# audeering/opensmile

Measured on NVIDIA H100. Metric: LLD frames/sec (16kHz, 25ms/10ms), higher is better.
Workload: dtype f32

## Files before the change

### opensmile_b200/csrc/lld_common.cuh

```cuda
#pragma once
#include <cstdio>

#include "fft_radix.cuh"
#include "kernels.cuh"

namespace osm {

struct SmemLayout {
  int zbuf, samp, raw, rawPcm, mbar, winLut, tw, splitTw, melCoef, melRange, dctCos, dctLift, eql, melS, ring;
  int total;
  int sampFloats, rawPcmBytes;
};

__host__ __device__ inline int align_up(int x, int a) { return (x + a - 1) / a * a; }

constexpr int kLeadFrames = 8;

__host__ __device__ inline SmemLayout make_layout(const LldParams &p, int M, int F)
{
  SmemLayout L;
  int o = 0;
  L.zbuf = o; o += M * F * 8;
  const int S = p.frameStep + p.sPad;
  L.sampFloats = align_up((F - 1) * S + p.frameSize + ((p.frameSize - 1) / p.frameStep) * p.sPad + 2, 4);
  L.samp = o; o += L.sampFloats * 4;
  L.raw = o; o += F * 4;
  o = align_up(o, 16);
  L.rawPcmBytes = align_up(16 + (kLeadFrames + (F - 1) * p.frameStep + p.frameSize) * p.nChan * 2, 16);
  L.rawPcm = o; o += L.rawPcmBytes;
  L.mbar = o; o += 16;
  L.winLut = o; o += M * 16;
  L.tw = o; o += p.twCount * 8;
  L.splitTw = o; o += (M / 2 + 1) * 8;
  o = align_up(o, 16);
  L.melCoef = o; o += (p.melVCount + 4) * 8;
  L.melRange = o; o += 2 * (p.nBands + 2) * 4;
  o = align_up(o, 16);
  L.dctCos = o; o += max(p.dctRows * p.dctStride, p.opKind == 0 ? p.nBands * 16 : 0) * 4;
  L.dctLift = o; o += p.nStat * 4;
  L.eql = o; o += (p.opKind == 1 ? p.nBands : 0) * 4;
  o = align_up(o, 16);
  if (L.sampFloats >= p.nBands * F) L.melS = L.samp;
  else { L.melS = o; o += p.nBands * F * 4; }
  L.ring = o; o += p.nStat * 2 * F * 4;
  L.total = align_up(o, 16);
  return L;
}

__device__ __forceinline__ float div32767(float x)
{
  const float rc = 3.0518509447574615e-05f;
  const float q0 = __fmul_rn(x, rc);
  const float r = __fmaf_rn(-q0, 32767.0f, x);
  return __fmaf_rn(r, rc, q0);
}

#define OSM_COLD __noinline__
template <bool F32>
__device__ __forceinline__ float pcm_to_float_generic(const int16_t *s, int nChan)
{
  if constexpr (F32) return *reinterpret_cast<const float *>(s);
  float tmp = (float)s[0];
  for (int c = 1; c < nChan; c++) tmp = __fadd_rn(tmp, (float)s[c]);
  if (nChan == 1) return div32767(tmp);
  if (nChan == 2) return div32767(tmp * 0.5f);
  return __fdiv_rn(__fdiv_rn(tmp, (float)nChan), 32767.0f);
}
template <bool F32>
static __device__ OSM_COLD float pcm_to_float_slow(const int16_t *s, int nChan) { return pcm_to_float_generic<F32>(s, nChan); }

__device__ __forceinline__ uint32_t smem_u32(const void *p) { return (uint32_t)__cvta_generic_to_shared(p); }

__device__ __forceinline__ void mbar_init(uint64_t *bar, int count)
{
  asm volatile("mbarrier.init.shared::cta.b64 [%0], %1;" ::"r"(smem_u32(bar)), "r"(count));
  asm volatile("fence.mbarrier_init.release.cluster;" ::: "memory");
}
__device__ __forceinline__ void mbar_expect_tx(uint64_t *bar, uint32_t bytes)
{
  asm volatile("mbarrier.arrive.expect_tx.shared::cta.b64 _, [%0], %1;" ::"r"(smem_u32(bar)), "r"(bytes) : "memory");
}
__device__ __forceinline__ void bulk_g2s(void *dst, const void *src, uint32_t bytes, uint64_t *bar)
{
  asm volatile("cp.async.bulk.shared::cluster.global.mbarrier::complete_tx::bytes [%0], [%1], %2, [%3];"
               ::"r"(smem_u32(dst)), "l"(src), "r"(bytes), "r"(smem_u32(bar)) : "memory");
}
__device__ __forceinline__ void mbar_wait(uint64_t *bar, uint32_t parity)
{
  asm volatile(
      "{\n"
      ".reg .pred p;\n"
      "LAB_WAIT:\n"
      "mbarrier.try_wait.parity.shared::cta.b64 p, [%0], %1;\n"
      "@p bra LAB_DONE;\n"
      "bra LAB_WAIT;\n"
      "LAB_DONE:\n"
      "}\n" ::"r"(smem_u32(bar)), "r"(parity) : "memory");
}

struct ChunkCtx {
  int utt, a, b;
  int T;
  int s0;
  int sEnd;
  int nT;
  int tile0;
  long long uo;
  long long row0;
};

template <int F>
__device__ __forceinline__ ChunkCtx load_chunk(const LldParams &p, int chunk)
{
  ChunkCtx c;
  const ChunkRef cr = p.chunks[chunk];
  c.utt = cr.utt; c.a = cr.a; c.b = cr.b; c.tile0 = cr.tile0;
  c.uo = p.uttOff[cr.utt];
  const long long Ls = p.uttOff[cr.utt + 1] - c.uo;
  c.T = (int)((Ls - p.frameSize) / p.frameStep + 1);
  c.s0 = max(cr.a - p.halo, 0);
  c.sEnd = min(cr.b + p.halo, c.T);
  c.nT = (c.sEnd - c.s0 + F - 1) / F;
  c.row0 = p.rowOff[cr.utt];
  return c;
}

__device__ __forceinline__ int chunk_run_begin(const LldParams &p, int g)
{
  const long long w = (long long)p.chunks[0].w0 + (long long)g * p.ctaTiles;
  int lo = 0, hi = p.nChunks;
  while (lo < hi) {
    const int mid = (lo + hi) >> 1;
    if (p.chunks[mid].w0 < w) lo = mid + 1;
    else hi = mid;
  }
  return lo;
}

struct TileGeom {
  int fs;
  int nf;
  int count;
  int lead;
  int mis;
  uint32_t bytes;
  const char *src;
};

template <int F>
__device__ __forceinline__ TileGeom tile_geom(const LldParams &p, const ChunkCtx &c, int j)
{
  TileGeom g;
  g.fs = c.s0 + j * F;
  g.nf = min(F, c.sEnd - g.fs);
  const long long s0 = (long long)g.fs * p.frameStep;
  g.count = (g.nf - 1) * p.frameStep + p.frameSize;
  g.lead = (s0 > 0) ? kLeadFrames : 0;
  const char *a = reinterpret_cast<const char *>(p.pcm + (c.uo + s0 - g.lead) * p.nChan);
  g.mis = (int)(reinterpret_cast<uintptr_t>(a) & 15);
  g.src = a - g.mis;
  g.bytes = (uint32_t)align_up(g.mis + (g.lead + g.count) * p.nChan * 2, 16);
  return g;
}

__device__ __forceinline__ float div_exact(float x, float d, float rcp)
{
  const float ax = fabsf(x);
  if (rcp != 0.f && ax > 1e-30f && ax < 1e30f) {
    const float q0 = __fmul_rn(x, rcp);
    const float r = __fmaf_rn(-q0, d, x);
    return __fmaf_rn(r, rcp, q0);
  }
  return __fdiv_rn(x, d);
}

__device__ __forceinline__ int win_navail(int t, int n0, int c0, int Tprev)
{
  return (t < c0) ? Tprev : min(n0 + (t - c0) + 1, Tprev);
}

template <int M, int F, int NVW, int R, int MS, bool FIRST, bool LAST, bool VEC2>
__device__ __forceinline__ void fft_stage(float2 *__restrict__ Z, const float *__restrict__ sampF,
                                          const float *__restrict__ raw,
                                          const float4 *__restrict__ winLut,
                                          const float2 *__restrict__ tw,
                                          const LldParams &p, int vw, int f)
{
  constexpr int stride = MS / R;
  for (int t = vw; t < M / R; t += NVW) {
    const int blk = t / stride, j = t % stride;
    const int base = blk * MS + j;
    float2 v[R];
    if (FIRST) {
#pragma unroll
      for (int r = 0; r < R; r++) {
        const float4 wl = winLut[base + stride * r];
        const int off = __float_as_int(wl.z);
        float2 x;
        if (VEC2) {
          x = *reinterpret_cast<const float2 *>(sampF + off);
        } else {
          x.x = sampF[off];
          x.y = sampF[off + 1];
        }
        v[r] = make_float2(__fmul_rn(x.x, wl.x), __fmul_rn(x.y, wl.y));
      }
      if (base == 0 && p.preemph)
        v[0].x = __fmul_rn(__fmul_rn(p.oneMinusK, raw[f]), winLut[0].x);
      if (p.hasWinOffset) {
#pragma unroll
        for (int r = 0; r < R; r++) {
          const float nv = winLut[base + stride * r].w;
          if (nv >= 1.f) v[r].x = __fadd_rn(v[r].x, p.winOffset);
          if (nv >= 2.f) v[r].y = __fadd_rn(v[r].y, p.winOffset);
        }
      }
    } else {
#pragma unroll
      for (int r = 0; r < R; r++) v[r] = Z[(base + stride * r) * F + f];
    }
    Dft<R>::run(v);
    if (!LAST) {
      const float2 *twj = tw + j * R;
#pragma unroll
      for (int q = 1; q < R; q++) v[Dft<R>::out(q)] = cmul(v[Dft<R>::out(q)], twj[q]);
    }
#pragma unroll
    for (int q = 0; q < R; q++) Z[(base + stride * q) * F + f] = v[Dft<R>::out(q)];
  }
}

constexpr int kMaxLp = 8;

template <int F, int NVW>
__device__ __forceinline__ void plp_backend(const LldParams &p, const float *melS, const float *sCos,
                                            const float *sLift, float *acfS, float *dst, int vw, int f)
{
  const int nB = p.nBands, nFreq = p.plpNFreq, nAuto = p.plpNAuto;
  if (!p.plpIDFT) {
    for (int i = vw; i < nB; i += NVW) dst[i * (2 * F) + f] = melS[i * F + f];
    return;
  }
  for (int i = vw; i < nAuto; i += NVW) {
    const float *ct = sCos + i * p.dctStride;
    double tmp = 0.0;
    if (p.plpHtk) tmp = (double)ct[0] * (double)melS[f];
    for (int m = 1; m < nFreq - 1; m++) tmp = __dadd_rn(tmp, (double)ct[m] * (double)melS[(m - 1) * F + f]);
    tmp = __dadd_rn(tmp, (double)ct[nFreq - 1] * (double)melS[(nFreq - 3) * F + f]);
    const float a = (float)(tmp / (2.0 * (double)(nFreq - 1)));
    if (!p.plpLP) dst[i * (2 * F) + f] = a;
    else acfS[i * F + f] = a;
  }
  if (!p.plpLP) return;
  __syncthreads();
  if (vw == 0) {
    const int P = p.plpOrder;
    float r[kMaxLp + 1], a[kMaxLp], cc[kMaxLp + 1];
#pragma unroll
    for (int i = 0; i <= kMaxLp; i++) r[i] = (i <= P) ? acfS[i * F + f] : 0.f;
#pragma unroll
    for (int i = 0; i < kMaxLp; i++) a[i] = 0.f;
    float gain = 0.f;
    if (r[0] != 0.f) {
      float e = r[0];
#pragma unroll
      for (int m = 1; m <= kMaxLp; m++) {
        if (m <= P && e != 0.f) {
          float sum = r[m];
#pragma unroll
          for (int i = 1; i < m; i++) sum = __fadd_rn(sum, __fmul_rn(a[i - 1], r[m - i]));
          const float km = __fmul_rn(__fdiv_rn(-1.0f, e), sum);
          a[m - 1] = km;
#pragma unroll
          for (int i = 1; i <= m / 2; i++) {
            const float x = a[i - 1];
            a[i - 1] = __fadd_rn(a[i - 1], __fmul_rn(km, a[m - i - 1]));
            if ((i < (m / 2)) || ((m & 1) == 1)) a[m - i - 1] = __fadd_rn(a[m - i - 1], __fmul_rn(km, x));
          }
          e = __fmul_rn(e, __fsub_rn(1.0f, __fmul_rn(km, km)));
        }
      }
      gain = e;
    }
    if (!p.plpCeps) {
#pragma unroll
      for (int i = 0; i < kMaxLp; i++) if (i < P) dst[i * (2 * F) + f] = a[i];
      return;
    }
    if (gain <= 0.f) gain = 1.0f;
    int first = p.plpFirstCC < 1 ? 1 : p.plpFirstCC;
    const int last = p.plpLastCC > P ? P : p.plpLastCC;
#pragma unroll
    for (int n = 1; n <= kMaxLp; n++) {
      if (n >= first && n <= last) {
        double sum = 0.0;
#pragma unroll
        for (int i = 1; i < n; i++)
          sum = __dadd_rn(sum, (double)__fmul_rn(__fmul_rn((float)(n - i), a[i - 1]), cc[n - i - 1]));
        cc[n - first] = -__fadd_rn(a[n - first], (float)(sum / (double)n));
      }
    }
    const float zeroth = (float)(-log(1.0 / (double)gain));
    const int nC = p.nStat;
#pragma unroll
    for (int i = 0; i <= kMaxLp; i++) {
      if (i < nC) {
        float v;
        if (p.plpFirstCC == 0) {
          if (p.plpHtk) v = (i == nC - 1) ? zeroth : cc[i];
          else v = (i == 0) ? zeroth : cc[i - 1];
        } else {
          v = cc[i];
        }
        if (p.plpLifter) v = __fmul_rn(v, sLift[i]);
        dst[i * (2 * F) + f] = v;
      }
    }
  }
}

template <int F, int NT>
__device__ __forceinline__ void emit_interior(const float *__restrict__ ring, float *__restrict__ Dbuf,
                                              float *__restrict__ outS, int K, int dRows, int slot0, int rslot0,
                                              float norm1, float rcp1, float norm2, float rcp2, int tid)
{
  const int K3 = 3 * K;
  constexpr int DR = F + 4;
  for (int item = tid; item < K * DR; item += NT) {
    const int c = item / DR, tt = item - c * DR;
    const float *rc = ring + c * (2 * F);
    const int sl = slot0 + tt;
    const float dA = __fsub_rn(rc[(sl + 1) & (2 * F - 1)], rc[(sl - 1) & (2 * F - 1)]);
    const float dB = __fsub_rn(rc[(sl + 2) & (2 * F - 1)], rc[(sl - 2) & (2 * F - 1)]);
    const float dv = div_exact(__fadd_rn(dA, __fmul_rn(2.0f, dB)), norm1, rcp1);
    Dbuf[c * dRows + tt] = dv;
    const int rr = tt - 2;
    if (rr >= 0 && rr < F) outS[rr * K3 + K + c] = dv;
  }
  for (int item = tid; item < K * F; item += NT) {
    const int c = item / F, rr = item - c * F;
    outS[rr * K3 + c] = ring[c * (2 * F) + ((rslot0 + rr) & (2 * F - 1))];
  }
  __syncthreads();
  for (int item = tid; item < K * F; item += NT) {
    const int c = item / F, rr = item - c * F;
    const float *dt = Dbuf + c * dRows + rr + 2;
    const float dA = __fsub_rn(dt[1], dt[-1]);
    const float dB = __fsub_rn(dt[2], dt[-2]);
    outS[rr * K3 + 2 * K + c] = div_exact(__fadd_rn(dA, __fmul_rn(2.0f, dB)), norm2, rcp2);
  }
  __syncthreads();
}

template <int F, int NW>
__device__ OSM_COLD void emit_edge(const float *__restrict__ ring, float *__restrict__ Dbuf, float *__restrict__ outS,
                               int K, int W1, int W2, int T, int T1, int c01, int c02, int s0, int r0, int r1,
                               int d0, int d1, int dRows, float norm1, float rcp1, float norm2, float rcp2,
                               int warp, int lane)
{
  const int K3 = 3 * K, nr = r1 - r0;
  for (int c = warp; c < K; c += NW) {
    const float *rc = ring + c * (2 * F);
    for (int tt = lane; tt < d1 - d0; tt += 32) {
      const int t = d0 + tt;
      float num = 0.f;
      for (int i = 1; i <= W1; i++) {
        const int hi = t + i, lo = t - i;
        float later, prior;
        if (t - W1 < 0) {
          later = (hi >= T) ? 0.f : rc[(hi - s0) & (2 * F - 1)];
          prior = rc[(max(lo, 0) - s0) & (2 * F - 1)];
        } else {
          later = rc[(min(hi, T - 1) - s0) & (2 * F - 1)];
          prior = rc[(min(lo, T - 1) - s0) & (2 * F - 1)];
        }
        num = __fadd_rn(num, __fmul_rn((float)i, __fsub_rn(later, prior)));
      }
      const float dv = div_exact(num, norm1, rcp1);
      Dbuf[c * dRows + tt] = dv;
      if (t >= r0 && t < r1) outS[(t - r0) * K3 + K + c] = dv;
    }
    for (int rr = lane; rr < nr; rr += 32) outS[rr * K3 + c] = rc[(r0 + rr - s0) & (2 * F - 1)];
  }
  __syncthreads();
  for (int c = warp; c < K; c += NW) {
    const float *dc = Dbuf + c * dRows - d0;
    for (int rr = lane; rr < nr; rr += 32) {
      const int t = r0 + rr;
      const int navail2 = win_navail(t, c01, c02, T1);
      float num = 0.f;
      for (int i = 1; i <= W2; i++) {
        const int hi = t + i, lo = t - i;
        float later, prior;
        if (t - W2 < 0) {
          later = (hi >= navail2) ? 0.f : dc[hi];
          prior = dc[max(lo, 0)];
        } else {
          later = dc[min(hi, navail2 - 1)];
          prior = dc[min(lo, navail2 - 1)];
        }
        num = __fadd_rn(num, __fmul_rn((float)i, __fsub_rn(later, prior)));
      }
      outS[rr * K3 + 2 * K + c] = div_exact(num, norm2, rcp2);
    }
  }
  __syncthreads();
}

}
```

### opensmile_b200/csrc/lld_fast.cu

```cuda
#include "lld_common.cuh"

namespace osm {

enum { kPhStage, kPhPass1, kPhPass2, kPhMel, kPhDct, kPhEmit, kPhStore, kPhKernel, kPhKernelMax, kPhTiles, kPhSlots };
#ifdef OSM_LLD_PHASE_CLOCKS
__device__ unsigned long long gLld512Phase[kPhSlots];
#define OSM_PHASE(k)                                                    \
  do {                                                                  \
    if (tid == 0) {                                                     \
      const long long c_ = clock64();                                   \
      sPh[k] += (unsigned long long)(c_ - phT);                         \
      phT = c_;                                                         \
    }                                                                   \
  } while (0)
#else
#define OSM_PHASE(k) do {} while (0)
#endif

namespace {

constexpr int kM = 256, kF = 32, kNT = 256, kNW = 8;
constexpr int kKMax = 16;
constexpr int kPartOff = 9216;

__device__ __forceinline__ void dft4_d0(float2 &a, float2 &b, float2 &c, float2 &d)
{
  const float2 t0 = cadd(a, c), t1 = csub(a, c), bb = b;
  a = cadd(t0, bb);
  c = csub(t0, bb);
  b = make_float2(t1.x + bb.y, t1.y - bb.x);
  d = make_float2(t1.x - bb.y, t1.y + bb.x);
}

template <int NZR>
__device__ __forceinline__ void dft16_first(float2 (&v)[16])
{
  dft4(v[0], v[4], v[8], v[12]);
  if (NZR <= 13) {
    dft4_d0(v[1], v[5], v[9], v[13]);
    dft4_d0(v[2], v[6], v[10], v[14]);
    dft4_d0(v[3], v[7], v[11], v[15]);
  } else {
    dft4(v[1], v[5], v[9], v[13]);
    dft4(v[2], v[6], v[10], v[14]);
    dft4(v[3], v[7], v[11], v[15]);
  }
  const float c1 = 0.92387953251128675613f, s1 = 0.38268343236508977173f;
  const float c2 = 0.70710678118654752440f;
  v[5] = cmul(v[5], make_float2(c1, -s1));
  { float2 a = v[6]; v[6] = make_float2(c2 * (a.x + a.y), c2 * (a.y - a.x)); }
  v[7] = cmul(v[7], make_float2(s1, -c1));
  { float2 a = v[9]; v[9] = make_float2(c2 * (a.x + a.y), c2 * (a.y - a.x)); }
  v[10] = cmul_mi(v[10]);
  { float2 a = v[11]; v[11] = make_float2(c2 * (a.y - a.x), -c2 * (a.x + a.y)); }
  v[13] = cmul(v[13], make_float2(s1, -c1));
  { float2 a = v[14]; v[14] = make_float2(c2 * (a.y - a.x), -c2 * (a.x + a.y)); }
  v[15] = cmul(v[15], make_float2(-c1, s1));
#pragma unroll
  for (int k1 = 0; k1 < 4; k1++) dft4(v[4 * k1], v[4 * k1 + 1], v[4 * k1 + 2], v[4 * k1 + 3]);
}

__device__ __forceinline__ void split_pair(float2 a, float2 b, float2 w, float &pk, float &pm)
{
  const float2 e2 = make_float2(a.x + b.x, a.y - b.y);
  const float2 o2 = make_float2(a.x - b.x, a.y + b.y);
  const float2 t2 = cmul(o2, w);
  const float xr = e2.x + t2.y, xi = e2.y - t2.x;
  const float yr = e2.x - t2.y, yi = e2.y + t2.x;
  pk = __fmaf_rn(xr, xr, __fmul_rn(xi, xi));
  pm = __fmaf_rn(yr, yr, __fmul_rn(yi, yi));
}

template <int NZR>
__global__ void __launch_bounds__(kNT, 2) lld512_kernel(const LldParams p)
{
  constexpr int M = kM, F = kF, NT = kNT, NW = kNW;
  using D16 = Dft<16>;

  extern __shared__ __align__(16) unsigned char smem[];
  __shared__ ChunkCtx sCx[2];
  __shared__ int sRun[2];
  const SmemLayout L = make_layout(p, M, F);
  float2 *Z = reinterpret_cast<float2 *>(smem + L.zbuf);
  float *P = reinterpret_cast<float *>(smem + L.zbuf);
  float *samp = reinterpret_cast<float *>(smem + L.samp);
  float *raw = reinterpret_cast<float *>(smem + L.raw);
  unsigned char *rawPcm = smem + L.rawPcm;
  uint64_t *mbar = reinterpret_cast<uint64_t *>(smem + L.mbar);
  float4 *sWinLut = reinterpret_cast<float4 *>(smem + L.winLut);
  float2 *sTw = reinterpret_cast<float2 *>(smem + L.tw);
  float2 *sSplit = reinterpret_cast<float2 *>(smem + L.splitTw);
  float2 *sMelCoef = reinterpret_cast<float2 *>(smem + L.melCoef);
  int *sMelRange = reinterpret_cast<int *>(smem + L.melRange);
  float *sDct = reinterpret_cast<float *>(smem + L.dctCos);
  float *sLift = reinterpret_cast<float *>(smem + L.dctLift);
  float *ring = reinterpret_cast<float *>(smem + L.ring);
  float *Dbuf = reinterpret_cast<float *>(smem + L.zbuf);

  const int tid = threadIdx.x;
  const int warp = tid >> 5, f = tid & 31;

  if (tid == 0) mbar_init(mbar, 1);
  if (tid < 2) sRun[tid] = chunk_run_begin(p, blockIdx.x + tid);
  for (int i = tid; i < M; i += NT) sWinLut[i] = p.winLut[i];
  for (int i = tid; i < p.twCount; i += NT) sTw[i] = p.twiddles[i];
  for (int i = tid; i < M / 2 + 1; i += NT) sSplit[i] = p.splitTw[i];
  for (int i = tid; i < p.melVCount; i += NT) sMelCoef[i] = p.melVisit[i];
  for (int i = tid; i < p.nBands + 2; i += NT) { sMelRange[i] = p.melRange[i]; sMelRange[p.nBands + 2 + i] = p.melVB[i]; }
  for (int i = tid; i < p.nBands * kKMax; i += NT) {
    const int m = i / kKMax, c = i - m * kKMax;
    sDct[i] = (c < p.nStat) ? p.dctCos[c * p.dctStride + m] : 0.f;
  }
  for (int i = tid; i < p.nStat; i += NT) sLift[i] = p.dctLift[i];
  for (int i = tid; i < L.sampFloats; i += NT) samp[i] = 0.f;
  for (int i = tid; i < F; i += NT) raw[i] = 0.f;
  __syncthreads();

  const int hop = p.frameStep;
  const int S = hop + p.sPad;
  uint32_t phase = 0;
#ifdef OSM_LLD_PHASE_CLOCKS
  __shared__ unsigned long long sPh[kPhSlots];
  if (tid < kPhSlots) sPh[tid] = 0;
  const long long phT0 = clock64();
  long long phT = phT0;
#endif

  int chunk = sRun[0];
  const int chunkEnd = sRun[1];
  if (chunk >= chunkEnd) return;
  int cpar = 0;
  if (tid == 0) {
    sCx[0] = load_chunk<F>(p, chunk);
    const TileGeom g0 = tile_geom<F>(p, sCx[0], 0);
    mbar_expect_tx(mbar, g0.bytes);
    bulk_g2s(rawPcm, g0.src, g0.bytes, mbar);
  }
  __syncthreads();
  int j = 0;
  int emitted = sCx[0].a;

  const int tA = (warp == 0) ? 0 : warp, tB = (warp == 0) ? 8 : 16 - warp;
  const int wl = (warp == 0) ? 8 : warp, wh = (warp == 0) ? 0 : warp;
  const int melBs = p.melSplit[warp], melBe = p.melSplit[warp + 1];

  while (chunk < chunkEnd) {
    const ChunkCtx &cx = sCx[cpar];

    mbar_wait(mbar, phase);
    phase ^= 1;
    {
      const TileGeom tg = tile_geom<F>(p, cx, j);
      const int count = tg.count;
      const int16_t *rp = reinterpret_cast<const int16_t *>(rawPcm + tg.mis) + tg.lead;
      const bool aligned = (tg.mis == 0);
      const bool hasLead = tg.lead > 0;
      const float ks = p.preDe ? p.preK : -p.preK;
#pragma unroll 1
      for (int i = tid * 8; i < count; i += NT * 8) {
        int wds[4];
        if (aligned) {
          const int4 w4 = *reinterpret_cast<const int4 *>(rp + i);
          wds[0] = w4.x; wds[1] = w4.y; wds[2] = w4.z; wds[3] = w4.w;
        } else {
          const unsigned short *up = reinterpret_cast<const unsigned short *>(rp + i);
#pragma unroll
          for (int jj = 0; jj < 4; jj++) wds[jj] = (int)((unsigned)up[2 * jj] | ((unsigned)up[2 * jj + 1] << 16));
        }
        float x[8], y[8];
#pragma unroll
        for (int jj = 0; jj < 4; jj++) {
          x[2 * jj] = div32767((float)(short)(wds[jj] & 0xffff));
          x[2 * jj + 1] = div32767((float)(wds[jj] >> 16));
        }
        if (p.preemph) {
          float xprev = 0.f;
          if (i > 0 || hasLead) xprev = div32767((float)rp[i - 1]);
#pragma unroll
          for (int jj = 0; jj < 8; jj++) y[jj] = __fadd_rn(x[jj], __fmul_rn(ks, (jj == 0) ? xprev : x[jj - 1]));
        } else {
#pragma unroll
          for (int jj = 0; jj < 8; jj++) y[jj] = x[jj];
        }
        const int q = (int)__umulhi((unsigned)i, p.hopMagic);
        float *dst = samp + i + q * p.sPad;
        if (i == q * hop && q < F) raw[q] = x[0];
#pragma unroll
        for (int jj = 0; jj < 8; jj += 2) *reinterpret_cast<float2 *>(dst + jj) = make_float2(y[jj], y[jj + 1]);
      }
    }
    __syncthreads();
    if (tid == 0) {
      if (j + 1 < cx.nT) {
        const TileGeom gn = tile_geom<F>(p, cx, j + 1);
        mbar_expect_tx(mbar, gn.bytes);
        bulk_g2s(rawPcm, gn.src, gn.bytes, mbar);
      } else if (chunk + 1 < chunkEnd) {
        const ChunkCtx cn = load_chunk<F>(p, chunk + 1);
        sCx[cpar ^ 1] = cn;
        const TileGeom gn = tile_geom<F>(p, cn, 0);
        mbar_expect_tx(mbar, gn.bytes);
        bulk_g2s(rawPcm, gn.src, gn.bytes, mbar);
      }
    }
    OSM_PHASE(kPhStage);

    {
      const float *sampF = samp + f * S;
      const float2 *tw0 = sTw + p.twOff[0];
#pragma unroll 1
      for (int t = warp; t < 16; t += NW) {
        float2 v[16];
#pragma unroll
        for (int r = 0; r < 16; r++) {
          if (r < NZR) {
            const float4 wl = sWinLut[t + 16 * r];
            const float2 x = *reinterpret_cast<const float2 *>(sampF + __float_as_int(wl.z));
            v[r] = make_float2(__fmul_rn(x.x, wl.x), __fmul_rn(x.y, wl.y));
          } else {
            v[r] = make_float2(0.f, 0.f);
          }
        }
        if (t == 0 && p.preemph)
          v[0].x = __fmul_rn(__fmul_rn(p.oneMinusK, raw[f]), sWinLut[0].x);
        dft16_first<NZR>(v);
        const float2 *twj = tw0 + t * 16;
#pragma unroll
        for (int q = 1; q < 16; q++) v[D16::out(q)] = cmul(v[D16::out(q)], twj[q]);
        float2 *zp = Z + t * F + f;
#pragma unroll
        for (int q = 0; q < 16; q++) zp[(16 * q) * F] = v[D16::out(q)];
      }
    }
    __syncthreads();
    OSM_PHASE(kPhPass1);

    {
      float2 A[16], v[16];
#pragma unroll 2
      for (int h = 0; h < 2; h++) {
        const float2 *zp = Z + ((h ? tB : tA) * 16) * F + f;
#pragma unroll
        for (int r = 0; r < 16; r++) v[r] = zp[r * F];
        D16::run(v);
        if (h == 0) {
#pragma unroll
          for (int r = 0; r < 16; r++) A[r] = v[r];
        }
      }
      const float2 x0 = A[D16::out(0)];
      if (warp == 0) {
        float2 na[8], nb[8];
#pragma unroll
        for (int q = 0; q < 8; q++) { na[q] = v[D16::out(q)]; nb[q] = A[D16::out(q + 1)]; }
#pragma unroll
        for (int q = 0; q < 8; q++) { A[D16::out(q)] = na[q]; v[D16::out(q)] = nb[q]; }
      }
      float pk[16], pm[16];
      {
        const float2 *swl = sSplit + wl, *swh = sSplit + (256 - wh);
#pragma unroll
        for (int q = 0; q < 16; q++) {
          const float2 aq = A[D16::out(q)], bq = v[D16::out(15 - q)];
          if (q < 8) split_pair(aq, bq, swl[16 * q], pk[q], pm[q]);
          else       split_pair(bq, aq, swh[-16 * q], pk[q], pm[q]);
        }
      }
      __syncthreads();
      {
        float *Plo = P + wl * F + f, *Plm = P + (256 - wl) * F + f;
        float *Phi = P + (256 - wh) * F + f, *Phm = P + wh * F + f;
#pragma unroll
        for (int q = 0; q < 8; q++) { Plo[(16 * q) * F] = pk[q]; Plm[(-16 * q) * F] = pm[q]; }
#pragma unroll
        for (int q = 8; q < 16; q++) {
          Phi[(-16 * q) * F] = pk[q];
          if (q > 8 || warp != 0) Phm[(16 * q) * F] = pm[q];
        }
      }
      if (warp == 0) {
        const float xr = 2.0f * (x0.x + x0.y), yr = 2.0f * (x0.x - x0.y);
        P[f] = __fmul_rn(xr, xr);
        P[M * F + f] = __fmul_rn(yr, yr);
      }
    }
    __syncthreads();
    OSM_PHASE(kPhPass2);

    float *melS = P + kPartOff;
    if (melBs < melBe) {
      const int *sVB = sMelRange + p.nBands + 2;
      float cur = 0.f;
      for (int r = melBs; r <= melBe; r++) {
        float nxt = 0.f;
        const float *pp = P + sMelRange[r] * F + f;
        const int v0 = sVB[r];
        const float4 *cp = reinterpret_cast<const float4 *>(sMelCoef + v0);
#pragma unroll 1
        for (int q = (sVB[r + 1] - v0) >> 2; q > 0; q--, pp += 4 * F, cp += 2) {
          const float p0 = pp[0], p1 = pp[F], p2 = pp[2 * F], p3 = pp[3 * F];
          const float4 wa = cp[0], wb = cp[1];
          cur = __fmaf_rn(p0, wa.x, cur); nxt = __fmaf_rn(p0, wa.y, nxt);
          cur = __fmaf_rn(p1, wa.z, cur); nxt = __fmaf_rn(p1, wa.w, nxt);
          cur = __fmaf_rn(p2, wb.x, cur); nxt = __fmaf_rn(p2, wb.y, nxt);
          cur = __fmaf_rn(p3, wb.z, cur); nxt = __fmaf_rn(p3, wb.w, nxt);
        }
        if (r > melBs) {
          float mval = __fmul_rn(cur, p.melScale);
          if (p.doLog) mval = (mval < p.melfloor) ? p.logMelfloor : logf(mval);
          melS[(r - 1) * F + f] = mval;
        }
        cur = nxt;
      }
    }
    __syncthreads();
    OSM_PHASE(kPhMel);

    const int ringBase = (j & 1) * F;
    {
      const int i = 2 * warp;
      if (i < p.nStat) {
        const float2 *cc = reinterpret_cast<const float2 *>(sDct + i);
        const float *lp = melS + f;
        float a0 = 0.f, a1 = 0.f;
#pragma unroll 4
        for (int m = 0; m < p.nBands; m++, lp += F, cc += kKMax / 2) {
          const float l0 = lp[0];
          const float2 c = cc[0];
          a0 = __fmaf_rn(l0, c.x, a0); a1 = __fmaf_rn(l0, c.y, a1);
        }
        ring[i * (2 * F) + ringBase + f] = __fmul_rn(a0, sLift[i]);
        if (i + 1 < p.nStat) ring[(i + 1) * (2 * F) + ringBase + f] = __fmul_rn(a1, sLift[i + 1]);
      }
    }
    __syncthreads();
    OSM_PHASE(kPhDct);

    const int tfs = cx.s0 + j * F;
    if (!p.fused) {
      const int tot = min(F, cx.sEnd - tfs) * p.nStat;
      for (int idx = tid; idx < tot; idx += NT) {
        const int ff = idx / p.nStat, c = idx - ff * p.nStat;
        p.out[(cx.row0 + tfs + ff) * p.outStride + p.outCol + c] = ring[c * (2 * F) + ringBase + ff];
      }
    } else {
      const int K = p.nStat, W1 = p.fW1, W2 = p.fW2, H = W1 + W2;
      const int T = cx.T;
      const int r0 = emitted;
      const int r1 = (j + 1 == cx.nT) ? cx.b : min(tfs + F - H, cx.b);
      const int T1 = T + W1, c01 = max(T - W1, 0), c02 = max(c01 - W2, 0);
      const float norm1 = p.fNorm1, norm2 = p.fNorm2;
      const int d0 = max(r0 - W2, 0), d1 = min(r1 + W2, T1);
      const int dRows = F + 24;
      float *outS = Dbuf + ((K * dRows + 3) & ~3);
      const int K3 = 3 * K;
      const int nr = r1 - r0;
      const bool interior1 = (d0 >= W1) && (d1 + W1 <= T);
      const bool interior2 = (r0 >= W2) && (r1 <= c02);
      if (interior1 && interior2 && W1 == 2 && W2 == 2 && nr == F) {
        emit_interior<F, NT>(ring, Dbuf, outS, K, dRows, d0 - cx.s0, r0 - cx.s0, norm1, p.fRcp1, norm2, p.fRcp2, tid);
      } else {
        emit_edge<F, NW>(ring, Dbuf, outS, K, W1, W2, T, T1, c01, c02, cx.s0, r0, r1, d0, d1, dRows, norm1, p.fRcp1, norm2, p.fRcp2, warp, f);
      }
      OSM_PHASE(kPhEmit);
      {
        float *o = p.out + (cx.row0 + r0) * (long long)K3;
        const int n = nr * K3;
        for (int i = tid; i < n; i += NT) o[i] = outS[i];
      }
      emitted = r1;
    }
    OSM_PHASE(kPhStore);
#ifdef OSM_LLD_PHASE_CLOCKS
    if (tid == 0) sPh[kPhTiles]++;
#endif

    j++;
    if (j == cx.nT) {
      chunk++;
      j = 0;
      cpar ^= 1;
      if (chunk < chunkEnd) emitted = sCx[cpar].a;
    }
  }
#ifdef OSM_LLD_PHASE_CLOCKS
  if (tid == 0) {
    sPh[kPhKernel] = (unsigned long long)(clock64() - phT0);
    for (int k = 0; k < kPhSlots; k++)
      if (k != kPhKernelMax) atomicAdd(&gLld512Phase[k], sPh[k]);
    atomicMax(&gLld512Phase[kPhKernelMax], sPh[kPhKernel]);
  }
#endif
}

template <int NZR>
cudaError_t launch_fast_t(const LldParams &p, int numSMs, cudaStream_t st, LldLaunchInfo *info, bool launch)
{
  const size_t smem = (size_t)make_layout(p, kM, kF).total;
  auto kern = lld512_kernel<NZR>;
  cudaError_t e = cudaFuncSetAttribute(kern, cudaFuncAttributeMaxDynamicSharedMemorySize, (int)smem);
  if (e != cudaSuccess) return e;
  int occ = 0;
  e = cudaOccupancyMaxActiveBlocksPerMultiprocessor(&occ, kern, kNT, smem);
  if (e != cudaSuccess) return e;
  if (occ < 1) return cudaErrorLaunchOutOfResources;
  const int grid = launch ? p.nRuns : numSMs * occ;
  if (info) {
    info->grid = grid; info->block = kNT; info->smem = smem; info->nChunks = p.nChunks;
    info->kernel = NZR == 13 ? "lld512_kernel<13>" : "lld512_kernel<16>";
  }
  if (!launch) return cudaSuccess;
  kern<<<grid, kNT, smem, st>>>(p);
  return cudaGetLastError();
}

}

bool lld_fast_applies(const LldParams &p, int nfft)
{
  return nfft == 512 && !p.narrow && p.opKind == 0 && p.magOut == nullptr && p.melUsePower && p.nChan == 1 &&
         p.frameStep % 8 == 0 && p.frameSize % 8 == 0 && p.frameSize <= 512 && !p.hasWinOffset && p.nStat <= kKMax &&
         ((p.frameStep + p.sPad) % 2) == 0;
}

cudaError_t launch_lld_fast(const LldParams &p, int numSMs, cudaStream_t st, LldLaunchInfo *info, bool launch)
{
  if (p.frameSize <= 416) return launch_fast_t<13>(p, numSMs, st, info, launch);
  return launch_fast_t<16>(p, numSMs, st, info, launch);
}

#ifdef OSM_LLD_PHASE_CLOCKS
extern "C" __attribute__((visibility("default"))) int osm_b200_lld512_phase_clocks(unsigned long long *out)
{
  cudaError_t e = cudaMemcpyFromSymbol(out, gLld512Phase, sizeof(gLld512Phase));
  if (e == cudaSuccess) {
    static const unsigned long long zero[kPhSlots] = {};
    e = cudaMemcpyToSymbol(gLld512Phase, zero, sizeof(zero));
  }
  return (int)e;
}
#endif

}
```

Baseline: 931.4 million.

## Store fused LLD output tiles with TMA bulk shared-to-global copies

The final output copy no longer has all threads loop over the tile writing floats to global memory. Thread 0 now issues a cp.async.bulk shared-to-global copy for the 16-byte-aligned middle, and the last warp writes the unaligned head and tail elements by hand. The staging buffer is offset to match the global address alignment, and a proxy fence plus a wait on bulk reads before the buffer is reused keep the asynchronous copy safe. This frees the threads to move on to the next tile while the store is in flight, at the cost of extra synchronisation and more complex alignment handling.

```diff
diff --git a/opensmile_b200/csrc/lld_common.cuh b/opensmile_b200/csrc/lld_common.cuh
--- a/opensmile_b200/csrc/lld_common.cuh
+++ b/opensmile_b200/csrc/lld_common.cuh
@@ -97,6 +97,15 @@
       "LAB_DONE:\n"
       "}\n" ::"r"(smem_u32(bar)), "r"(parity) : "memory");
 }
+__device__ __forceinline__ void fence_proxy_async_smem() { asm volatile("fence.proxy.async.shared::cta;" ::: "memory"); }
+__device__ __forceinline__ void bulk_s2g(void *dst, const void *src, uint32_t bytes)
+{
+  asm volatile("cp.async.bulk.global.shared::cta.bulk_group [%0], [%1], %2;"
+               ::"l"(dst), "r"(smem_u32(src)), "r"(bytes) : "memory");
+  asm volatile("cp.async.bulk.commit_group;" ::: "memory");
+}
+__device__ __forceinline__ void bulk_wait_read() { asm volatile("cp.async.bulk.wait_group.read 0;" ::: "memory"); }
+__device__ __forceinline__ void bulk_wait() { asm volatile("cp.async.bulk.wait_group 0;" ::: "memory"); }
 
 struct ChunkCtx {
   int utt, a, b;
@@ -319,7 +328,7 @@
   }
 }
 
-template <int F, int NT>
+template <int F, int NT, bool BULK_OUT = false>
 __device__ __forceinline__ void emit_interior(const float *__restrict__ ring, float *__restrict__ Dbuf,
                                               float *__restrict__ outS, int K, int dRows, int slot0, int rslot0,
                                               float norm1, float rcp1, float norm2, float rcp2, int tid)
@@ -349,10 +358,11 @@
     const float dB = __fsub_rn(dt[2], dt[-2]);
     outS[rr * K3 + 2 * K + c] = div_exact(__fadd_rn(dA, __fmul_rn(2.0f, dB)), norm2, rcp2);
   }
+  if (BULK_OUT) fence_proxy_async_smem();
   __syncthreads();
 }
 
-template <int F, int NW>
+template <int F, int NW, bool BULK_OUT = false>
 __device__ OSM_COLD void emit_edge(const float *__restrict__ ring, float *__restrict__ Dbuf, float *__restrict__ outS,
                                int K, int W1, int W2, int T, int T1, int c01, int c02, int s0, int r0, int r1,
                                int d0, int d1, int dRows, float norm1, float rcp1, float norm2, float rcp2,
@@ -404,6 +414,7 @@
       outS[rr * K3 + 2 * K + c] = div_exact(num, norm2, rcp2);
     }
   }
+  if (BULK_OUT) fence_proxy_async_smem();
   __syncthreads();
 }
 
diff --git a/opensmile_b200/csrc/lld_fast.cu b/opensmile_b200/csrc/lld_fast.cu
--- a/opensmile_b200/csrc/lld_fast.cu
+++ b/opensmile_b200/csrc/lld_fast.cu
@@ -189,6 +189,7 @@
         for (int jj = 0; jj < 8; jj += 2) *reinterpret_cast<float2 *>(dst + jj) = make_float2(y[jj], y[jj + 1]);
       }
     }
+    if (tid == 0) bulk_wait_read();
     __syncthreads();
     if (tid == 0) {
       if (j + 1 < cx.nT) {
@@ -352,21 +353,28 @@
       const float norm1 = p.fNorm1, norm2 = p.fNorm2;
       const int d0 = max(r0 - W2, 0), d1 = min(r1 + W2, T1);
       const int dRows = F + 24;
-      float *outS = Dbuf + ((K * dRows + 3) & ~3);
       const int K3 = 3 * K;
+      float *o = p.out + (cx.row0 + r0) * (long long)K3;
+      const int res = (int)((reinterpret_cast<uintptr_t>(o) >> 2) & 3);
+      float *outS = Dbuf + ((K * dRows + 3) & ~3) + res;
       const int nr = r1 - r0;
       const bool interior1 = (d0 >= W1) && (d1 + W1 <= T);
       const bool interior2 = (r0 >= W2) && (r1 <= c02);
       if (interior1 && interior2 && W1 == 2 && W2 == 2 && nr == F) {
-        emit_interior<F, NT>(ring, Dbuf, outS, K, dRows, d0 - cx.s0, r0 - cx.s0, norm1, p.fRcp1, norm2, p.fRcp2, tid);
+        emit_interior<F, NT, true>(ring, Dbuf, outS, K, dRows, d0 - cx.s0, r0 - cx.s0, norm1, p.fRcp1, norm2, p.fRcp2, tid);
       } else {
-        emit_edge<F, NW>(ring, Dbuf, outS, K, W1, W2, T, T1, c01, c02, cx.s0, r0, r1, d0, d1, dRows, norm1, p.fRcp1, norm2, p.fRcp2, warp, f);
+        emit_edge<F, NW, true>(ring, Dbuf, outS, K, W1, W2, T, T1, c01, c02, cx.s0, r0, r1, d0, d1, dRows, norm1, p.fRcp1, norm2, p.fRcp2, warp, f);
       }
       OSM_PHASE(kPhEmit);
       {
-        float *o = p.out + (cx.row0 + r0) * (long long)K3;
-        const int n = nr * K3;
-        for (int i = tid; i < n; i += NT) o[i] = outS[i];
+        const int n = max(nr, 0) * K3;
+        const int hd = min((4 - res) & 3, n), mid = (n - hd) & ~3, tl = n - hd - mid;
+        if (tid == 0 && mid > 0) bulk_s2g(o + hd, outS + hd, (uint32_t)mid * 4);
+        if (tid >= NT - 32) {
+          const int i = tid - (NT - 32);
+          if (i < hd) o[i] = outS[i];
+          else if (i >= 4 && i - 4 < tl) o[hd + mid + i - 4] = outS[hd + mid + i - 4];
+        }
       }
       emitted = r1;
     }
@@ -383,6 +391,7 @@
       if (chunk < chunkEnd) emitted = sCx[cpar].a;
     }
   }
+  if (tid == 0) bulk_wait();
 #ifdef OSM_LLD_PHASE_CLOCKS
   if (tid == 0) {
     sPh[kPhKernel] = (unsigned long long)(clock64() - phT0);
```

New measurement: 950.5 million, median of 6. 2.1% higher.

## Use warp-shuffle deltas for interior emit, vectorize aligned output stores, rotate staging writes

Applied to the files above, without the earlier changes.

The interior emit path is replaced by a warp-per-coefficient routine that computes first-order deltas once per lane and gets the second-order delta neighbours through warp shuffles plus a small halo, instead of going through a shared delta buffer. The staged output is shifted by the global pointer's misalignment so the copy to global memory can use float4 stores with scalar handling at the edges. Per-thread float2 stores into the sample buffer are rotated by thread index to spread shared-memory bank conflicts. In exchange there is more index arithmetic and an extra __syncthreads after the interior emit, and the halo lane mapping assumes K is at most 16.

```diff
diff --git a/opensmile_b200/csrc/lld_fast.cu b/opensmile_b200/csrc/lld_fast.cu
--- a/opensmile_b200/csrc/lld_fast.cu
+++ b/opensmile_b200/csrc/lld_fast.cu
@@ -69,6 +69,41 @@
   const float yr = e2.x - t2.y, yi = e2.y + t2.x;
   pk = __fmaf_rn(xr, xr, __fmul_rn(xi, xi));
   pm = __fmaf_rn(yr, yr, __fmul_rn(yi, yi));
+}
+
+__device__ __forceinline__ void emit_lanes(const float *__restrict__ ring, float *__restrict__ outS, int K, int rslot0,
+                                           float norm1, float rcp1, float norm2, float rcp2, int warp, int lane)
+{
+  constexpr int F = kF, RM = 2 * F - 1;
+  const int K3 = 3 * K;
+  const auto delta = [&](const float *rc, int s) {
+    const float dA = __fsub_rn(rc[(s + 1) & RM], rc[(s - 1) & RM]);
+    const float dB = __fsub_rn(rc[(s + 2) & RM], rc[(s - 2) & RM]);
+    return div_exact(__fadd_rn(dA, __fmul_rn(2.0f, dB)), norm1, rcp1);
+  };
+  const int e = lane & 3;
+  const float halo = delta(ring + min(warp + 8 * ((lane >> 2) & 1), K - 1) * (2 * F), rslot0 + (e < 2 ? e - 2 : e + 30));
+  const int srcA = (lane & 1) + ((lane >> 3) & 2), srcB = 1 + (lane >> 4);
+#pragma unroll
+  for (int h = 0; h < 2; h++) {
+    const int c = warp + 8 * h;
+    if (c >= K) break;
+    const float *rc = ring + c * (2 * F);
+    const int s = rslot0 + lane;
+    const float x = rc[s & RM];
+    const float dv = delta(rc, s);
+    const float up1 = __shfl_up_sync(0xffffffffu, dv, 1), up2 = __shfl_up_sync(0xffffffffu, dv, 2);
+    const float dn1 = __shfl_down_sync(0xffffffffu, dv, 1), dn2 = __shfl_down_sync(0xffffffffu, dv, 2);
+    const float hA = __shfl_sync(0xffffffffu, halo, 4 * h + srcA), hB = __shfl_sync(0xffffffffu, halo, 4 * h + srcB);
+    const float m1 = (lane == 0) ? hB : up1, m2 = (lane < 2) ? hA : up2;
+    const float p1 = (lane == 31) ? hB : dn1, p2 = (lane >= 30) ? hA : dn2;
+    const float dA = __fsub_rn(p1, m1);
+    const float dB = __fsub_rn(p2, m2);
+    float *o = outS + lane * K3 + c;
+    o[0] = x;
+    o[K] = dv;
+    o[2 * K] = div_exact(__fadd_rn(dA, __fmul_rn(2.0f, dB)), norm2, rcp2);
+  }
 }
 
 template <int NZR>
@@ -185,8 +220,16 @@
         const int q = (int)__umulhi((unsigned)i, p.hopMagic);
         float *dst = samp + i + q * p.sPad;
         if (i == q * hop && q < F) raw[q] = x[0];
-#pragma unroll
-        for (int jj = 0; jj < 8; jj += 2) *reinterpret_cast<float2 *>(dst + jj) = make_float2(y[jj], y[jj + 1]);
+        {
+          float2 pr[4];
+#pragma unroll
+          for (int k = 0; k < 4; k++) pr[k] = make_float2(y[2 * k], y[2 * k + 1]);
+          const int rot = (tid >> 2) & 3;
+          if (rot & 1) { const float2 t = pr[0]; pr[0] = pr[1]; pr[1] = pr[2]; pr[2] = pr[3]; pr[3] = t; }
+          if (rot & 2) { float2 t = pr[0]; pr[0] = pr[2]; pr[2] = t; t = pr[1]; pr[1] = pr[3]; pr[3] = t; }
+#pragma unroll
+          for (int k = 0; k < 4; k++) *reinterpret_cast<float2 *>(dst + 2 * ((k + rot) & 3)) = pr[k];
+        }
       }
     }
     __syncthreads();
@@ -352,21 +395,35 @@
       const float norm1 = p.fNorm1, norm2 = p.fNorm2;
       const int d0 = max(r0 - W2, 0), d1 = min(r1 + W2, T1);
       const int dRows = F + 24;
-      float *outS = Dbuf + ((K * dRows + 3) & ~3);
       const int K3 = 3 * K;
       const int nr = r1 - r0;
+      float *o = p.out + (cx.row0 + r0) * (long long)K3;
+      const int mis = (int)((reinterpret_cast<uintptr_t>(o) >> 2) & 3);
+      float *outA = Dbuf + ((K * dRows + 3) & ~3);
+      float *outS = outA + mis;
       const bool interior1 = (d0 >= W1) && (d1 + W1 <= T);
       const bool interior2 = (r0 >= W2) && (r1 <= c02);
       if (interior1 && interior2 && W1 == 2 && W2 == 2 && nr == F) {
-        emit_interior<F, NT>(ring, Dbuf, outS, K, dRows, d0 - cx.s0, r0 - cx.s0, norm1, p.fRcp1, norm2, p.fRcp2, tid);
+        emit_lanes(ring, outS, K, r0 - cx.s0, norm1, p.fRcp1, norm2, p.fRcp2, warp, f);
+        __syncthreads();
       } else {
         emit_edge<F, NW>(ring, Dbuf, outS, K, W1, W2, T, T1, c01, c02, cx.s0, r0, r1, d0, d1, dRows, norm1, p.fRcp1, norm2, p.fRcp2, warp, f);
       }
       OSM_PHASE(kPhEmit);
       {
-        float *o = p.out + (cx.row0 + r0) * (long long)K3;
         const int n = nr * K3;
-        for (int i = tid; i < n; i += NT) o[i] = outS[i];
+        const float4 *s4 = reinterpret_cast<const float4 *>(outA);
+        float4 *g4 = reinterpret_cast<float4 *>(o - mis);
+        for (int v = tid; v < (mis + n + 3) >> 2; v += NT) {
+          const int lo = 4 * v - mis;
+          if (lo >= 0 && lo + 4 <= n) {
+            g4[v] = s4[v];
+          } else {
+#pragma unroll
+            for (int e = 0; e < 4; e++)
+              if (lo + e >= 0 && lo + e < n) o[lo + e] = outS[lo + e];
+          }
+        }
       }
       emitted = r1;
     }
```

Measured after the change: 935.0 million before, 951.1 million after (median of 6 runs). +1.7%, better.
